# rvolden/C3POa

Hardware: AMD Instinct MI355X
Metric: R2C2 reads->consensus/sec (higher is better)
Workload: dtype int32

## Files before the change

### c3poa_amd/csrc/c3_api.hip

```cpp
#include "c3_dev.h"
#include "c3_args.h"
#include "c3_bgzf.h"
#include "c3_fastq.h"
#include "c3_inflate.h"
#include <algorithm>
#include <cstddef>
#include <cstdio>
#include <cstring>
#include <string>
#include <vector>

extern "C" void c3k_launch_conk(const ConkArgs*, int, int, int, hipStream_t);
extern "C" void c3k_launch_adapter(const AdapterArgs*, int, hipStream_t);
extern "C" void c3k_launch_pairwise(const uint8_t*, int, const uint8_t*, int, const uint8_t*, int, uint8_t*, uint8_t*, int*, hipStream_t);
extern "C" void c3k_launch_match_index(const char*, const int*, int, int, const char*, const long long*, int*, hipStream_t);
extern "C" void c3k_launch_demux(const uint8_t*, int, const uint8_t*, int, int, int, int32_t*, uint8_t*, hipStream_t);
extern "C" void c3k_launch_peaks(const PeaksArgs*, int, hipStream_t);
extern "C" int c3k_peaks_blocks_per_cu(void);
extern "C" void c3k_launch_poa(const PoaArgs*, int, int, int, hipStream_t);
extern "C" void c3k_launch_prep(const PrepArgs*, int, hipStream_t);
extern "C" void c3k_launch_window(const WinArgs*, int, hipStream_t);
extern "C" void c3k_launch_stitch(const StitchArgs*, int, hipStream_t);
extern "C" void c3k_launch_zero(const ZeroArgs*, int, hipStream_t);
extern "C" void c3k_launch_zero_long(const ZeroArgs*, int, hipStream_t);
// ... 494 lines not shown
  }
  HIPCHK(hipMemcpyAsync(h->d_zwork.p, h->zwork.data(), sizeof(int) * (size_t)nz, hipMemcpyHostToDevice, h->stream));
  if (ns) {
    ZeroArgs z; fill_zero_args(h, z, ns); z.dcap = dmax;
    DBG("zero: nz=%d grid=%d dmax=%lld\n", ns, std::min(ns, 512), dmax);
    c3k_launch_zero(&z, std::min(ns, 512), h->stream);
    HIPCHK(hipGetLastError());
  }
  if (nl) {
    ZeroArgs z; fill_zero_args(h, z, nl);
    z.work = h->d_zwork.as<int>() + ns; z.S = h->s_zero_l.as<uint8_t>(); z.scap = smax; z.zk = zk;
    DBG("zero long: nz=%d grid=%d slot=%lld K=%d\n", nl, grid_l, smax, zk);
    c3k_launch_zero_long(&z, grid_l, h->stream);
    HIPCHK(hipGetLastError());
  }
  { int r_ = copy_summary(h); DBG("zero done\n"); return r_; }
}

static int fetch_summary(c3_handle* h) {
  int rc = copy_summary(h);
  DBG("summary copied\n");
  if (rc) return rc;
  const auto wl0 = std::chrono::steady_clock::now();
  struct WlTimer { c3_handle* h; std::chrono::steady_clock::time_point t0; ~WlTimer() { h->tm.ms_host_worklist = std::chrono::duration<float, std::milli>(std::chrono::steady_clock::now() - t0).count(); } } wl_timer_{h, wl0};
  HIPCHK(zero_cnt(h, &dev_cnt(h)->zero_cells));
  if ((rc = run_zero(h))) return rc;
  const int n = h->n;
  h->work.clear();
  for (int i = 0; i < n; ++i) if (h->sum[i].status == C3_ST_OK && h->sum[i].n_sub >= 1) h->work.push_back(i);
  if (n < (1 << 24)) {
    const size_t m = h->work.size();
    std::vector<uint64_t> keys(m), tmp(m);
    for (size_t k = 0; k < m; ++k) {
      const int i = h->work[k];
      const uint64_t cost = (uint64_t)h->sum[i].sum_sub * (uint64_t)h->sum[i].n_sub;
      keys[k] = ((((uint64_t)1 << 40) - 1 - cost) << 24) | (uint64_t)i;
    }
    uint64_t* src = keys.data(); uint64_t* dst = tmp.data();
    for (int pass = 0; pass < 4; ++pass) {
      const int sh = 24 + 10 * pass;
      size_t cnt[1025] = {0};
      for (size_t k = 0; k < m; ++k) ++cnt[((src[k] >> sh) & 1023) + 1];
      for (int b = 0; b < 1024; ++b) cnt[b + 1] += cnt[b];
      for (size_t k = 0; k < m; ++k) dst[cnt[(src[k] >> sh) & 1023]++] = src[k];
      std::swap(src, dst);
    }
    for (size_t k = 0; k < m; ++k) h->work[k] = (int)(src[k] & 0xffffff);
  } else {
    std::stable_sort(h->work.begin(), h->work.end(), [&](int x, int y) {
      long cx = (long)h->sum[x].sum_sub * h->sum[x].n_sub, cy = (long)h->sum[y].sum_sub * h->sum[y].n_sub; return cx > cy; });
  }
  HIPCHK(h->d_work.ensure(sizeof(int) * std::max<size_t>(h->work.size(), 1)));
  if (!h->work.empty()) HIPCHK(hipMemcpyAsync(h->d_work.p, h->work.data(), sizeof(int) * h->work.size(), hipMemcpyHostToDevice, h->stream));
  return 0;
}

static int launch_poa(c3_handle* h, const int* d_work, int nw, int Ncap, int K, int Pcap, long long cells, int* d_overflow, int* d_overflow16, int waves_per_cu, int wide_ring) {
  cells = (cells + 15) & ~15LL;
  cells = (cells + 63) & ~63LL;
  const bool w32 = d_overflow16 == nullptr || getenv("C3_DEBUG_POA32");
  const PoaLayout L = c3_poa_layout(Ncap, K, (int)cells, c3_poa_far_shift(w32), Pcap);
  const int slots = auto_slots(h, h->cfg.slots_poa, L.total, nw, waves_per_cu);
  const size_t S = (size_t)slots;
  HIPCHK(h->s_poa_i.ensure(L.ints * S)); HIPCHK(h->s_poa_nk.ensure(L.edges * S));
  HIPCHK(h->s_poa_cells.ensure(L.cells * S + 256)); HIPCHK(h->s_poa_b.ensure(L.bases * S)); HIPCHK(h->s_poa_sc.ensure(L.score * S));
  HIPCHK(h->s_poa_desc.ensure(L.desc * S)); HIPCHK(h->s_poa_jump.ensure(L.jump * S)); HIPCHK(h->s_poa_path.ensure(L.path * S));
  PoaArgs a; memset(&a, 0, sizeof(a));
  a.b = dev_batch(h); a.info = h->d_info.as<C3Info>(); a.p = dev_params(h->cfg);
  a.cnt = dev_cnt(h); a.work = d_work; a.n_work = nw;
  a.ibase = h->s_poa_i.as<int>(); a.ebase = h->s_poa_nk.as<int>(); a.cellsb = h->s_poa_cells.as<char>();
  a.bbase = h->s_poa_b.as<uint8_t>(); a.score = h->s_poa_sc.as<long long>();
  a.Ncap = Ncap; a.K = K; a.Pcap = Pcap; a.cells_cap = (int)cells; a.desc = h->s_poa_desc.as<uint4>(); a.jump = h->s_poa_jump.as<int>();
  a.pbase = h->s_poa_path.as<int>(); a.overflow = d_overflow; a.overflow16 = d_overflow16;
  if (const char* e = getenv("C3_DEBUG_POA_RBSPAN")) a.rb_span = std::max(3300, atoi(e));
  a.no2col = getenv("C3_DEBUG_POA_NO2COL") != nullptr;
  a.draft = h->d_draft.as<uint8_t>(); a.tpos = h->d_tpos.as<int32_t>();
  a.msa_dbg = nullptr; a.msa_off = nullptr; a.msa_len = nullptr;
  if (h->debug_msa) { a.msa_dbg = h->d_msa.as<uint8_t>(); a.msa_off = h->d_msa_off.as<int64_t>(); a.msa_len = h->d_msa_len.as<int>(); }
  DBG("poa: nw=%d Ncap=%d K=%d cells=%lld slots=%d (%.1f MB per slot)%s\n", nw, Ncap, K, cells, slots, L.total / 1048576.0, d_overflow ? "" : (d_overflow16 ? " [full-size pass]" : " [32-bit pass]"));
  c3k_launch_poa(&a, slots, w32 ? 1 : 0, wide_ring, h->stream);
  HIPCHK(hipGetLastError());
  return 0;
}

static int run_poa(c3_handle* h) {
  const int nw = (int)h->work.size();
  HIPCHK(h->d_draft.ensure((size_t)h->total + 64)); HIPCHK(h->d_tpos.ensure(sizeof(int32_t) * (size_t)h->total + 64));
  HIPCHK(h->d_cons.ensure((size_t)h->total + 64));
  HIPCHK(hipMemsetAsync(h->d_tpos.p, 0xff, sizeof(int32_t) * (size_t)h->total, h->stream));
  if (nw == 0) return 0;
  int max_sum = 0, max_ns = 0, max_q = 0;
  for (int i : h->work) { max_sum = std::max(max_sum, h->sum[i].sum_sub); max_ns = std::max(max_ns, h->sum[i].n_sub); max_q = std::max(max_q, h->sum[i].max_sub); }
  const int Ncap_full = max_sum + 8, K = max_ns + 1, Pcap = max_sum + 8;
  const int w = h->cfg.poa_band_b + (int)(h->cfg.poa_band_f * max_q);
  long long cells_full = (long long)(2 * max_q + 2) * (2 * w + 1 + max_q / 5);
  if (max_ns < 2) cells_full = 64;
  if (cells_full > 0x7fffff00LL) cells_full = 0x7fffff00LL;
  const double nodes_typ = (double)max_q * (1.0 + 0.15 * std::max(0, max_ns - 1));
  int Ncap = (int)std::min<double>(Ncap_full, 1.3 * nodes_typ + 256);
  long long cells = std::min<long long>(cells_full, (long long)(1.5 * nodes_typ * (2 * w + 12)) + 4096);
  if (const char* e_ = getenv("C3_DEBUG_POA_SMALL")) { Ncap = std::min(Ncap_full, std::max(64, atoi(e_))); cells = std::min<long long>(cells_full, 16LL * Ncap); }
  if (h->debug_msa) {
    std::vector<int64_t> mo(h->n + 1, 0);
    for (int i = 0; i < h->n; ++i) mo[i + 1] = mo[i] + (int64_t)h->sum[i].n_sub * (h->sum[i].sum_sub + 2);
    HIPCHK(h->d_msa.ensure((size_t)mo[h->n] + 64)); HIPCHK(h->d_msa_off.ensure(sizeof(int64_t) * (h->n + 1))); HIPCHK(h->d_msa_len.ensure(sizeof(int) * h->n));
    HIPCHK(hipMemcpyAsync(h->d_msa_off.p, mo.data(), sizeof(int64_t) * (h->n + 1), hipMemcpyHostToDevice, h->stream));
    HIPCHK(hipMemsetAsync(h->d_msa_len.p, 0, sizeof(int) * h->n, h->stream));
    HIPCHK(hipStreamSynchronize(h->stream));
  }
  HIPCHK(h->d_overflow.ensure(sizeof(int) * 2 * (size_t)nw));
  C3Counters* dc = dev_cnt(h);
  HIPCHK(zero_cnt(h, &dc->queue)); HIPCHK(zero_cnt(h, &dc->cells)); HIPCHK(zero_cnt(h, &dc->poa_ovf)); HIPCHK(zero_cnt(h, &dc->poa_ovf16));
  HIPCHK(zero_cnt(h, &dc->phases));
  int wide_ring = (max_q > 1792 || 2 * w + 1 + 24 > 128) ? 1 : 0;
  if (const char* e_ = getenv("C3_DEBUG_POA_WIDE")) wide_ring = atoi(e_) ? 1 : 0;
  int* ovA = h->d_overflow.as<int>(); int* ovB = h->d_overflow.as<int>() + nw;
  int rc = launch_poa(h, h->d_work.as<int>(), nw, Ncap, K, Pcap, cells, ovA, ovB, 24, wide_ring);
  if (rc) return rc;
  h->n_poa_redo = 0; h->n_poa_redo16 = 0;
  C3Counters c;
  HIPCHK(read_counters(h, &c));
  if (c.poa_ovf > 0) {
    h->n_poa_redo = c.poa_ovf;
    HIPCHK(zero_cnt(h, &dc->queue));
    if ((rc = launch_poa(h, ovA, c.poa_ovf, Ncap_full, K, Pcap, cells_full, nullptr, ovB, 24, wide_ring))) return rc;
    HIPCHK(read_counters(h, &c));
  }
  if (c.poa_ovf16 > 0) {
    h->n_poa_redo += c.poa_ovf16; h->n_poa_redo16 = c.poa_ovf16;
    HIPCHK(zero_cnt(h, &dc->queue));
    if ((rc = launch_poa(h, ovB, c.poa_ovf16, Ncap_full, K, Pcap, cells_full, nullptr, nullptr, 24, 0))) return rc;
  }
  if (!h->zwork.empty()) {
    ZeroArgs z; fill_zero_args(h, z, (int)h->zwork.size());
    c3k_launch_zero_finish(&z, std::min((int)h->zwork.size(), 512), h->stream);
    HIPCHK(hipGetLastError());
  }
  HIPCHK(hipMemcpyAsync(h->phase_poa, dc->phases, sizeof(h->phase_poa), hipMemcpyDeviceToHost, h->stream));
  return 0;
}

static int run_polish(c3_handle* h, float* ms_prep, float* ms_win, float* ms_st) {
  const int nw = (int)h->work.size();
  DBG("polish: nw=%d\n", nw);
  HIPCHK(h->d_cons.ensure((size_t)h->total + 64));
  if (nw == 0) return 0;
  const int WL = h->cfg.pol_window;
  int max_ns = 0, max_q = 0, max_dang = 0; long long wcap = 0;
  for (int i : h->work) {
    max_ns = std::max(max_ns, h->sum[i].n_sub); max_q = std::max(max_q, h->sum[i].max_sub); max_dang = std::max(max_dang, h->sum[i].max_dang);
    wcap += (2 * h->sum[i].max_sub + WL - 1) / WL + 1;
  }
  const int NLcap = max_ns + 2, NWcap = (2 * max_q + WL - 1) / WL + 1;
  const int64_t ecap = (int64_t)(max_dang + 2) * 512;
  const size_t per_slot_prep = (size_t)ecap + (size_t)NLcap * NWcap * 8;
  const int slots_p = auto_slots(h, h->cfg.slots_poa, per_slot_prep, nw, getenv("C3_DEBUG_PREP_WPC") ? atoi(getenv("C3_DEBUG_PREP_WPC")) : 20);
  HIPCHK(h->s_eD.ensure((size_t)ecap * slots_p));
  HIPCHK(h->s_lw.ensure(sizeof(int) * (size_t)NLcap * NWcap * 2 * slots_p));
  HIPCHK(h->d_wrec.ensure(sizeof(WinRec) * (size_t)wcap)); HIPCHK(h->d_wlay.ensure(sizeof(WLayer) * (size_t)wcap * NLcap));
  HIPCHK(h->d_wbase.ensure(sizeof(int) * (size_t)h->n));
  PrepArgs p; memset(&p, 0, sizeof(p));
  p.b = dev_batch(h); p.info = h->d_info.as<C3Info>(); p.p = dev_params(h->cfg);
  p.cnt = dev_cnt(h); p.work = h->d_work.as<int>(); p.n_work = nw;
  p.draft = h->d_draft.as<uint8_t>(); p.tpos = h->d_tpos.as<int32_t>();
  p.eD = h->s_eD.as<uint8_t>(); p.ecap = ecap;
  p.lw_first = h->s_lw.as<int>(); p.lw_last = p.lw_first + (size_t)NLcap * NWcap * slots_p; p.NLcap = NLcap; p.NWcap = NWcap;
  p.wrec = h->d_wrec.as<WinRec>(); p.wlay = h->d_wlay.as<WLayer>(); p.win_base = h->d_wbase.as<int>();
  p.wcap = (int)std::min<long long>(wcap, 0x7fffffff);
  HIPCHK(zero_counters(h));
  HIPCHK(hipEventRecord(h->ev[5], h->stream));
  DBG("prep: slots=%d ecap=%lld NL=%d NW=%d wcap=%lld\n", slots_p, (long long)ecap, NLcap, NWcap, (long long)wcap);
  c3k_launch_prep(&p, slots_p, h->stream);
  HIPCHK(hipGetLastError());
  HIPCHK(hipEventRecord(h->ev[6], h->stream));
  C3Counters c;
  HIPCHK(read_counters(h, &c));
  h->tm.cells_polish += c.cells; h->tm.cells_polish_computed += c.cells;
  const int n_win = (int)std::min<long long>(c.n_windows, std::min<long long>(wcap, 0x7fffffff));
  h->n_windows = n_win;
  DBG("prep done: n_win=%d\n", n_win);
  const int wout_cap = 3 * WL + 64;
  HIPCHK(hipEventRecord(h->ev[7], h->stream));
  if (n_win > 0) {
    HIPCHK(h->d_wout.ensure((size_t)n_win * wout_cap));
    const int Ncap = 3 * WL + 40 * NLcap, K = NLcap + 2;
    const long long hcap_full = (long long)(Ncap + 1) * 64 * 12;
    const int R_typ = std::min(Ncap, WL + WL / 4 + 30 * NLcap + 64);
    long long hcap = std::min(hcap_full, (long long)(R_typ + R_typ / 2 + 4) * 256);
    if (const char* e = getenv("C3_DEBUG_HCAP_DIV")) hcap = std::max(4096LL, hcap_full / std::max(1, atoi(e)) / 64 * 64);
    const WinLayout L = c3_win_layout(Ncap, K, hcap), L2 = c3_win_layout(Ncap, K, hcap_full);
    const int slots = auto_slots(h, h->cfg.slots_win, L.total, n_win, 20);
    const int slots2 = hcap < hcap_full ? std::min(slots, 256) : 0;
    const size_t S = (size_t)slots, S2 = (size_t)slots2;
    HIPCHK(h->s_win_i.ensure(L.ints * S + 64)); HIPCHK(h->s_win_nk.ensure(L.edges * S));
    HIPCHK(h->s_win_h.ensure(L.H * S)); HIPCHK(h->s_win_d.ensure(L.D * S + 256));
    HIPCHK(h->s_win_b.ensure(L.bases * S)); HIPCHK(h->s_win_sc.ensure(L.score * S)); HIPCHK(h->s_win_desc.ensure(L.desc * S));
    if (slots2) {
      HIPCHK(h->s_win_h2.ensure(L2.H * S2)); HIPCHK(h->s_win_d2.ensure(L2.D * S2 + 256));
      HIPCHK(h->d_wovf.ensure(sizeof(int) * (size_t)n_win));
    }
    WinArgs a; memset(&a, 0, sizeof(a));
    a.b = dev_batch(h); a.p = dev_params(h->cfg); a.cnt = dev_cnt(h); a.n_win = n_win;
    a.wrec_in = h->d_wrec.as<WinRec>(); a.wrec = h->d_wrec.as<WinRec>(); a.wlay = h->d_wlay.as<WLayer>(); a.NLcap = NLcap;
    a.draft = h->d_draft.as<uint8_t>();
    a.ibase = h->s_win_i.as<int>(); a.ebase = h->s_win_nk.as<int>();
    a.base = h->s_win_b.as<uint8_t>(); a.score = h->s_win_sc.as<long long>();
    a.H = h->s_win_h.as<int32_t>(); a.D = h->s_win_d.as<uint16_t>(); a.rdesc = h->s_win_desc.as<uint4>(); a.Ncap = Ncap; a.K = K; a.hcap = hcap; a.Lcap = std::min(std::min(Ncap, 2 * WL + 30 * NLcap), ((getenv("C3_DEBUG_WIN_LDS") ? atoi(getenv("C3_DEBUG_WIN_LDS")) : 6656) - 16) / 6);
    if (const char* e = getenv("C3_DEBUG_WIN_LCAP")) a.Lcap = std::max(64, std::min(Ncap, atoi(e)));
    a.wout = h->d_wout.as<uint8_t>(); a.wout_cap = wout_cap;
    HIPCHK(zero_counters(h));
    if (const char* e = getenv("C3_DEBUG_BAND")) a.band_mode = !strcmp(e, "off") ? 1 : !strcmp(e, "fail") ? 2 : !strcmp(e, "verify") ? 3 : 0;
    a.ovf_list = slots2 ? h->d_wovf.as<int>() : nullptr;
    c3k_launch_window(&a, slots, h->stream);
    HIPCHK(hipGetLastError());
    if (slots2) {
      a.H = h->s_win_h2.as<int32_t>(); a.D = h->s_win_d2.as<uint16_t>(); a.hcap = hcap_full;
      a.wlist = h->d_wovf.as<int>(); a.ovf_list = nullptr;
      c3k_launch_window(&a, slots2, h->stream);
      HIPCHK(hipGetLastError());
    }
    HIPCHK(hipMemcpyAsync(h->phase_win, dev_cnt(h)->phases, sizeof(h->phase_win), hipMemcpyDeviceToHost, h->stream));
  }
  HIPCHK(hipEventRecord(h->ev[8], h->stream));
  StitchArgs s; memset(&s, 0, sizeof(s));
  s.b = dev_batch(h); s.info = h->d_info.as<C3Info>(); s.work = h->d_work.as<int>(); s.n_work = nw;
  s.wrec = h->d_wrec.as<WinRec>(); s.win_base = h->d_wbase.as<int>(); s.wout = h->d_wout.as<uint8_t>(); s.wout_cap = wout_cap;
  s.cons = h->d_cons.as<char>(); s.zflag = h->d_zflag.as<uint8_t>();
  DBG("stitch\n");
  c3k_launch_stitch(&s, std::min(nw, h->n_cus * 16), h->stream);
  HIPCHK(hipGetLastError());
  HIPCHK(hipEventRecord(h->ev[9], h->stream));
  HIPCHK(read_counters(h, &c));
  if (n_win > 0) {
    h->tm.n_win_redo = c.win_ovf; h->tm.cells_polish += c.cells; h->tm.cells_polish_computed += c.cells_computed;
    h->tm.n_band_layers = c.band_layers; h->tm.n_band_fallback = c.band_fallback; h->tm.n_band_mismatch = c.band_mismatch;
    if (c.band_mismatch) fprintf(stderr, "c3poa: band verify mismatch in window %d layer %d (R = %d): last differing base q = %d, band row %d, full row %d, row of q+1 = %d\n",
                                 c.verify.window, c.verify.layer, c.verify.R, c.verify.q, c.verify.band_row, c.verify.full_row, c.verify.next_row);
  }
  HIPCHK(hipEventElapsedTime(ms_prep, h->ev[5], h->ev[6]));
  HIPCHK(hipEventElapsedTime(ms_win, h->ev[7], h->ev[8]));
  HIPCHK(hipEventElapsedTime(ms_st, h->ev[8], h->ev[9]));
  h->tm.n_windows = n_win;
  return 0;
}

static const long long QV_BUDGET = 1LL << 30;
static int qv_scratch(c3_handle* h, long long max_m, long long max_n, int n_items, QvArgs& a, int* grid) {
  a.dir_words = (max_m + 7) / 8 * 64;
  a.lds_n = (int)std::min<long long>((max_n + 15) / 16 * 16, c3k_qv_lds_max());
  a.gcap = max_n > a.lds_n ? (max_n + 15) / 16 * 16 : 0;
  const long long per_wg = 4 * 4 * a.dir_words + 5 * a.gcap;
  *grid = (int)std::max(1LL, std::min<long long>(std::min(n_items, h->n_cus * 8), QV_BUDGET / per_wg));
  HIPCHK(h->s_qv_dirs.ensure(sizeof(uint32_t) * (size_t)a.dir_words * 4 * (size_t)*grid + 256));
  if (a.gcap) HIPCHK(h->s_qv_g.ensure((size_t)a.gcap * 5 * (size_t)*grid + 256));
  a.dirs = h->s_qv_dirs.as<uint32_t>();
  a.gS = a.gcap ? h->s_qv_g.as<int>() : nullptr; a.gcodes = a.gcap ? h->s_qv_g.as<uint8_t>() + (size_t)a.gcap * 4 * (size_t)*grid : nullptr;
  HIPCHK(h->d_qv_cnt.ensure(64));
  HIPCHK(hipMemsetAsync(h->d_qv_cnt.p, 0, 64, h->stream));
  a.cnt = h->d_qv_cnt.as<unsigned long long>();
  return 0;
}
static int qv_counts(c3_handle* h, float ms) {
  unsigned long long c[8];
  HIPCHK(hipMemcpyAsync(c, h->d_qv_cnt.p, 64, hipMemcpyDeviceToHost, h->stream));
  HIPCHK(hipStreamSynchronize(h->stream));
  h->qtm.ms_qv = ms; h->qtm.n_reads = (int64_t)c[0]; h->qtm.n_pieces = (int64_t)c[1]; h->qtm.n_skipped = (int64_t)c[2];
  h->qtm.band_cells = (int64_t)c[3]; h->qtm.edge_hits = (int64_t)c[4];
  return 0;
}

static int run_qv(c3_handle* h) {
  for (int i = 0; i < 2; ++i) if (!h->ev_qv[i]) HIPCHK(hipEventCreate(&h->ev_qv[i]));
  HIPCHK(h->d_qv.ensure((size_t)h->total + 64));
  QvArgs a; memset(&a, 0, sizeof(a));
  int grid = 0;
  int rc = qv_scratch(h, h->maxL, h->maxL, h->n, a, &grid);
  if (rc) return rc;
  a.n_reads = h->n; a.info = h->d_info.as<C3Info>(); a.pk = h->d_pk.as<uint32_t>(); a.woff = h->d_woff.as<int64_t>();
  a.qual = h->d_qual.as<uint8_t>(); a.off = h->d_off.as<int64_t>(); a.cons = h->d_cons.as<char>(); a.qv = h->d_qv.as<char>();
  a.sa_np = -1;
  DBG("qv: grid=%d dir_words=%lld lds_n=%d gcap=%lld\n", grid, a.dir_words, a.lds_n, a.gcap);
  HIPCHK(hipEventRecord(h->ev_qv[0], h->stream));
  c3k_launch_qv(&a, grid, h->stream);
  HIPCHK(hipGetLastError());
  HIPCHK(hipEventRecord(h->ev_qv[1], h->stream));
  HIPCHK(hipEventSynchronize(h->ev_qv[1]));
  float ms = 0; HIPCHK(hipEventElapsedTime(&ms, h->ev_qv[0], h->ev_qv[1]));
  return qv_counts(h, ms);
}

extern "C" int c3_batch_run(c3_handle* h, int stages) {
  if (!h || h->n <= 0) return C3_E_STATE;
  if ((stages & C3_STAGE_QV) && !((stages | h->stages_done) & C3_STAGE_POLISH))
    return c3_fail(h, C3_E_STATE, "C3_STAGE_QV needs the polish stage (in this call or an earlier one on the resident batch)");
  HIPCHK(hipSetDevice(h->cfg.device));
  int rc;
  float ms;
  hipEvent_t t0 = h->ev[0], t1 = h->ev[1], t2 = h->ev[2], t3 = h->ev[3], t4 = h->ev[4];
  DBG("run: start n=%d\n", h->n);
  const auto wall0 = std::chrono::steady_clock::now();
  const double alloc0 = g_alloc_ms;
  if (stages & C3_STAGE_CONK) { h->tm.ms_conk = 0; h->tm.cells_conk = 0; }
  if (stages & C3_STAGE_PEAKS) h->tm.ms_peaks = 0;
  if (stages & C3_STAGE_POA) { h->tm.ms_poa = 0; h->tm.cells_poa = 0; }
  if (stages & C3_STAGE_POLISH) { h->tm.ms_prep = h->tm.ms_window = h->tm.ms_stitch = 0; h->tm.cells_polish = 0; h->tm.cells_polish_computed = 0; h->tm.n_band_layers = h->tm.n_band_fallback = h->tm.n_band_mismatch = 0; h->tm.n_windows = 0; h->tm.n_win_redo = 0; }
  HIPCHK(hipEventRecord(t0, h->stream));
  if (stages & C3_STAGE_CONK) { if ((rc = run_conk(h))) return rc; h->tm.cells_conk = 0; for (int i = 0; i < h->n; ++i) h->tm.cells_conk += (h->off[i + 1] - h->off[i]) * (int64_t)h->max_spl; }
// ... 915 lines not shown
```

### c3poa_amd/csrc/k_polish.hip

```cpp
#include "c3_dev.h"
#include "c3_args.h"
#include <algorithm>

#define WSYNC() __syncthreads()
#define EI(v, k) ((size_t)(k) * (size_t)c.Ncap + (size_t)(v))
#ifndef C3_WIN_RING
#define C3_WIN_RING 1
#endif



#ifndef C3_PREP_WAVES
#define C3_PREP_WAVES 5
#endif
#define EC 5
#define EXT_DCAP 4096
template <bool DL>
__device__ long long extend_align(const PrepArgs& a, const uint32_t* pk, const uint8_t* draft, const uint8_t* ldraft, int C,
                                  int pb, int n, int dir_, int32_t* tpos, uint8_t* D, int lane) {
  const int W = a.p.dang_band, bw = 2 * W + 1;
  const int mt4 = a.p.pol_match * 4, mm4 = a.p.pol_mismatch * 4, g4 = a.p.pol_gap * 4;
  const int db = dir_ > 0 ? 0 : C - 1;
  const int NEGK = -(1 << 28);
  for (int k = lane; k < n; k += 64) tpos[pb + dir_ * k] = -1;
  if (bw > 64 * EC || (long long)(n + 1) * 512 > a.ecap) return -1;
  int hprev[EC];
#pragma unroll
  for (int cc = 0; cc < EC; ++cc) {
    const int bb = lane * EC + cc, j = bb - W;
    hprev[cc] = (bb < bw && j >= 0 && j <= C) ? j * g4 : NEGK;
  }
  int best = 0, bi = 0, bj = 0;
  long long cells = lane == 0 ? min(C, W) + 1 : 0;
#ifndef C3_EXT_OLD
  if (DL) {
    const int bb0 = lane * EC;
    int g4bb1[EC], bestc[EC], bic[EC];
#pragma unroll
    for (int cc = 0; cc < EC; ++cc) { g4bb1[cc] = g4 * (bb0 + cc) + 1; bestc[cc] = 0; bic[cc] = 0; }
    auto code_at = [&](int q) { return (unsigned)ldraft[db + dir_ * min(max(q, 0), C - 1)]; };
    unsigned dcp = 0;
#pragma unroll
    for (int cc = 0; cc < EC; ++cc) dcp |= code_at(1 - W + bb0 + cc - 1) << (4 * cc);
    long long cells_s = 0;
    for (int ib = 1; ib <= n; ib += 64) {
      int pcs = 0;
      if (ib + lane <= n) pcs = c3_code_at(pk, pb + dir_ * (ib + lane - 1));
      asm volatile("" : "+v"(pcs));
      const int cnt = min(64, n - ib + 1);
      for (int li = 0; li < cnt; ++li) {
        const int i = ib + li;
        const int pc = __builtin_amdgcn_readlane(pcs, li);
        const unsigned nxt_code = code_at(i - W + bb0 + EC - 1);
        const int vlo = W - i;
        const int vhi = min(bw - 1, C - i + W);
        const unsigned span = (unsigned)(vhi - vlo);
        cells_s += max(0, vhi - max(0, vlo) + 1);
        const int nxt0 = __builtin_amdgcn_update_dpp(NEGK, hprev[0], 0x130, 0xf, 0xf, false);
        int key[EC], y[EC];
        int run = NEGK;
#pragma unroll
        for (int cc = 0; cc < EC; ++cc) {
          const int dcode = (int)((dcp >> (4 * cc)) & 15u);
          const int kd = hprev[cc] + ((pc == dcode) ? mt4 + 3 : mm4 + 3);
          const int up = (cc + 1 < EC) ? hprev[cc + 1 < EC ? cc + 1 : cc] : nxt0;
          const int k = max(kd, up + (g4 + 2));
          const bool val = (unsigned)(bb0 + cc - vlo) <= span && vhi >= vlo && bb0 + cc >= 0;
          key[cc] = val ? k : NEGK;
          y[cc] = (key[cc] & ~3) - (g4bb1[cc] - 1);
          run = max(run, y[cc]);
        }
        const int s = wave_scan_max(run);
        int ex = wave_shr1(s, NEGK);
        unsigned d0 = 0, d1 = 0;
#pragma unroll
        for (int cc = 0; cc < EC; ++cc) {
          int k2 = max(key[cc], ex + g4bb1[cc]);
          ex = max(ex, y[cc]);
          k2 = key[cc] == NEGK ? NEGK : k2;
          const int hh = k2 & ~3;
          hprev[cc] = hh;
          const unsigned tag = (unsigned)k2 & 3u;
          if (cc < 4) d0 |= tag << (8 * cc); else d1 |= tag;
          const bool up_ = hh > bestc[cc];
          bestc[cc] = max(bestc[cc], hh);
          bic[cc] = up_ ? i : bic[cc];
        }
        unsigned* drow = (unsigned*)(D + (size_t)i * 512) + lane * 2;
        drow[0] = 0x03030303u - d0; drow[1] = 3u - d1;
        dcp = (dcp >> 4) | (nxt_code << (4 * (EC - 1)));
      }
    }
#pragma unroll
    for (int cc = 0; cc < EC; ++cc) {
      const bool better = bestc[cc] > best || (bestc[cc] == best && bestc[cc] > 0 && bic[cc] < bi);
      if (better) { best = bestc[cc]; bi = bic[cc]; bj = bic[cc] - W + bb0 + cc; }
    }
    cells += lane == 0 ? cells_s : 0;
  } else
#endif
  for (int ib = 1; ib <= n; ib += 64) {
    int pcs = 0;
    if (ib + lane <= n) pcs = c3_code_at(pk, pb + dir_ * (ib + lane - 1));
    asm volatile("" : "+v"(pcs));
    const int cnt = min(64, n - ib + 1);
    for (int li = 0; li < cnt; ++li) {
      const int i = ib + li;
      const int pc = __builtin_amdgcn_readlane(pcs, li);
      const int jlo = max(0, i - W);
      const int nxt0 = __builtin_amdgcn_update_dpp(NEGK, hprev[0], 0x130, 0xf, 0xf, false);
      int key[EC], y[EC];
      int run = NEGK;
#pragma unroll
      for (int cc = 0; cc < EC; ++cc) {
        const int bb = lane * EC + cc, j = i - W + bb;
        const bool val = bb < bw && j >= 0 && j <= C;
        int k = INT32_MIN;
        if (val) {
          if (j > 0) {
            const int dcode = DL ? (int)ldraft[db + dir_ * (j - 1)] : (int)draft[db + dir_ * (j - 1)];
            k = hprev[cc] + ((pc == dcode) ? mt4 : mm4) + 3;
          }
          const int up = (cc + 1 < EC) ? hprev[cc + 1 < EC ? cc + 1 : cc] : nxt0;
          if (bb + 1 < bw) k = max(k, up + g4 + 2);
        }
        key[cc] = val ? k : NEGK;
        y[cc] = val ? (k & ~3) - g4 * bb : NEGK;
        run = max(run, y[cc]);
      }
      const int s = wave_scan_max(run);
      int ex = wave_shr1(s, NEGK);
      unsigned d0 = 0, d1 = 0;
#pragma unroll
      for (int cc = 0; cc < EC; ++cc) {
        const int bb = lane * EC + cc, j = i - W + bb;
        const bool val = bb < bw && j >= 0 && j <= C;
        int k2 = key[cc];
        if (val && j > jlo) k2 = max(k2, ex + g4 * bb + 1);
        ex = max(ex, y[cc]);
        const int hh = k2 & ~3;
        hprev[cc] = val ? hh : NEGK;
        const unsigned dir = val ? (unsigned)(3 - (k2 & 3)) : 3u;
        if (cc < 4) d0 |= dir << (8 * cc); else d1 |= dir;
        if (val) { ++cells; if (j > 0 && hh > best) { best = hh; bi = i; bj = j; } }
      }
      unsigned* drow = (unsigned*)(D + (size_t)i * 512) + lane * 2;
      drow[0] = d0; drow[1] = d1;
    }
  }
  WSYNC();
  const int gb = wave_max(best);
  const int gi = wave_min(best == gb ? bi : INT32_MAX / 2);
  const int gj = wave_min((best == gb && bi == gi) ? bj : INT32_MAX / 2);
  if (gb > 0) {
    int i = gi, j = gj;
    while (i > 0 || j > 0) {
      if (i == 0) break;
      const int bb = j - i + W;
      const int ik = i - lane;
      int d = 3;
      if (ik >= 1) d = D[(size_t)ik * 512 + (bb / EC) * 8 + bb % EC];
      const unsigned long long bal = __ballot(ik >= 1 && d == 0 && j - lane >= 1);
      const int m = (~bal) ? __builtin_ctzll(~bal) : 64;
      if (lane < m) tpos[pb + dir_ * (ik - 1)] = db + dir_ * (j - lane - 1);
      i -= m; j -= m;
      if (m < 64 && i > 0) {
        const int dbk = wave_bcast(d, m);
        if (dbk == 1) --i; else if (dbk == 2) --j; else break;
      }
    }
  }
  WSYNC();
  long long tot = cells;
  for (int o = 32; o > 0; o >>= 1) tot += __shfl_xor(tot, o);
  return tot;
}

__device__ __forceinline__ void prep_one(const PrepArgs& a, int wi, int lane, uint8_t* ldraft, uint8_t* eD, int* lwf, int* lwl, int WL) {
    const int rid = a.work[wi];
    C3Info* info = &a.info[rid];
    if (info->status != C3_ST_OK || info->draft_len <= 0) { info->n_win = 0; a.win_base[rid] = 0; return; }
    const int64_t off = a.b.off[rid];
    const int L = (int)(a.b.off[rid + 1] - off);
    const uint32_t* pk = a.b.pk + a.b.woff[rid];
    const uint8_t* qual = a.b.qual + off;
    const uint8_t* draft = a.draft + off;
    int32_t* tpos = a.tpos + off;
    const int C = info->draft_len, ns = info->n_sub;
    const int hf = info->has_front, ht = info->has_tail;
    long long cells = 0;
    if ((ht || hf) && C <= EXT_DCAP) { for (int t = lane; t < C; t += 64) ldraft[t] = draft[t]; WSYNC(); }
#ifdef C3_EXP_X2_EXT
    if (C <= EXT_DCAP) {
      if (ht) { long long r = extend_align<true>(a, pk, draft, ldraft, C, info->tail_beg, L - info->tail_beg, +1, tpos, eD, lane); if (r > 1LL << 60) cells += r; }
      if (hf) { long long r = extend_align<true>(a, pk, draft, ldraft, C, info->front_end - 1, info->front_end, -1, tpos, eD, lane); if (r > 1LL << 60) cells += r; }
    }
#endif
    if (C <= EXT_DCAP) {
      if (ht) { long long r = extend_align<true>(a, pk, draft, ldraft, C, info->tail_beg, L - info->tail_beg, +1, tpos, eD, lane); if (r > 0) cells += r; }
      if (hf) { long long r = extend_align<true>(a, pk, draft, ldraft, C, info->front_end - 1, info->front_end, -1, tpos, eD, lane); if (r > 0) cells += r; }
    } else {
      if (ht) { long long r = extend_align<false>(a, pk, draft, ldraft, C, info->tail_beg, L - info->tail_beg, +1, tpos, eD, lane); if (r > 0) cells += r; }
      if (hf) { long long r = extend_align<false>(a, pk, draft, ldraft, C, info->front_end - 1, info->front_end, -1, tpos, eD, lane); if (r > 0) cells += r; }
    }
    const int nl = ns + hf + ht;
    const int nwin = (C + WL - 1) / WL;
    if (nwin > a.NWcap || nl > a.NLcap) { info->status = C3_ST_LIMIT; info->n_win = 0; a.win_base[rid] = 0; return; }
    long tl = 0;
    for (int i = 0; i < nl; ++i) {
      int lb, le;
      if (i < ns) { lb = info->sub_beg[i]; le = info->sub_end[i]; }
      else if (i == ns && hf) { lb = 0; le = info->front_end; }
      else { lb = info->tail_beg; le = L; }
      tl += le - lb;
    }
    const int tgs = tl > 1000L * nl;
    int wbase = 0;
    if (lane == 0) wbase = atomicAdd(&a.cnt->n_windows, nwin);
    wbase = wave_first(wbase);
    if (wbase + nwin > a.wcap) {
      for (int w = lane; w < nwin && wbase + w < a.wcap; w += 64) {
        WinRec r; r.rid = rid; r.w = w; r.n_layers = 0; r.blen = 0; r.tgs = 0; r.out_len = 0; r.polished = 0; r.pad_ = 0;
        a.wrec[wbase + w] = r;
      }
      info->status = C3_ST_LIMIT; info->n_win = 0; a.win_base[rid] = 0; return;
    }
    for (int i = lane; i < nl * nwin; i += 64) { lwf[i] = INT32_MAX; lwl[i] = -1; }
    for (int w = lane; w < nwin; w += 64) {
      WinRec r; r.rid = rid; r.w = w; r.n_layers = 0; r.blen = (w * WL + WL <= C) ? WL : C - w * WL; r.tgs = tgs; r.out_len = 0; r.polished = 0; r.pad_ = 0;
      a.wrec[wbase + w] = r;
    }
    WSYNC();
    for (int i = 0; i < nl; ++i) {
      int lb, le;
      if (i < ns) { lb = info->sub_beg[i]; le = info->sub_end[i]; }
      else if (i == ns && hf) { lb = 0; le = info->front_end; }
      else { lb = info->tail_beg; le = L; }
      int qf = INT32_MAX, ql = -1;
      for (int k0 = lb; k0 < le; k0 += 64) {
        const int k = k0 + lane;
        const int t = k < le ? tpos[k] : -1;
        const bool valid = t >= 0;
        const int w = valid ? t / WL : -1;
        const unsigned long long vm = __ballot(valid);
        const unsigned long long below = vm & ((1ull << lane) - 1ull);
        const unsigned long long above = lane == 63 ? 0ull : (vm & ~((2ull << lane) - 1ull));
        const int pl = below ? 63 - __builtin_clzll(below) : lane, nx = above ? __builtin_ctzll(above) : lane;
        const int wp = __shfl(w, pl), wn = __shfl(w, nx);
        if (valid) {
          qf = min(qf, k); ql = max(ql, k);
          if (!below || wp != w) atomicMin(&lwf[i * nwin + w], k);
          if (!above || wn != w) atomicMax(&lwl[i * nwin + w], k);
        }
      }
      qf = wave_min(qf); ql = wave_max(ql);
      WSYNC();
      if (ql < 0) continue;
      const int qs = ql + 1 - qf, ts = tpos[ql] + 1 - tpos[qf];
      const double err = 1.0 - (double)min(qs, ts) / (double)max(qs, ts);
      if (err > 0.3) continue;
      for (int w = 0; w < nwin; ++w) {
        const int fq = lwf[i * nwin + w], lq = lwl[i * nwin + w];
        if (lq < 0) continue;
        const int seglen = lq + 1 - fq;
        if ((double)seglen < 0.02 * WL) continue;
        long qsum = 0;
        for (int x = fq + lane; x <= lq; x += 64) qsum += (int)qual[x] - 33;
        for (int o = 32; o > 0; o >>= 1) qsum += __shfl_xor(qsum, o);
        if (qsum < (long)a.p.pol_q * seglen) continue;
        if (lane == 0) {
          WinRec* r = &a.wrec[wbase + w];
          WLayer* dst = &a.wlay[(size_t)(wbase + w) * a.NLcap + r->n_layers];
          dst->qbeg = fq; dst->len = seglen; dst->begin = tpos[fq] - w * WL; dst->end = tpos[lq] - w * WL;
          r->n_layers++;
        }
      }
      WSYNC();
    }
    if (lane == 0) {
      info->n_win = nwin; a.win_base[rid] = wbase;
      atomicAdd(&a.cnt->cells, (unsigned long long)cells);
    }
    WSYNC();
}

__global__ __launch_bounds__(64, C3_PREP_WAVES) void k_prep(PrepArgs a) {
  const int lane = wave_lane();
  const int slot = blockIdx.x;
  __shared__ uint8_t ldraft[EXT_DCAP];
  uint8_t* eD = a.eD + (size_t)slot * a.ecap;
  int* lwf = a.lw_first + (size_t)slot * a.NLcap * a.NWcap;
  int* lwl = a.lw_last + (size_t)slot * a.NLcap * a.NWcap;
  const int WL = a.p.pol_window;
  for (;;) {
    int wi = 0;
    if (lane == 0) wi = atomicAdd(&a.cnt->queue, 1);
    wi = wave_first(wi);
    if (wi >= a.n_work) break;
    prep_one(a, wi, lane, ldraft, eD, lwf, lwl, WL);
  }
}


template <class T> struct WArr {
  T* base; unsigned off;
  __device__ __forceinline__ T& at(unsigned i) const { return *(T*)((char*)base + ((i + off) * (unsigned)sizeof(T))); }
  __device__ __forceinline__ T& operator[](int i) const { return at((unsigned)i); }
  __device__ __forceinline__ T& operator[](unsigned i) const { return at(i); }
  __device__ __forceinline__ T& operator[](long long i) const { return at((unsigned)i); }
  __device__ __forceinline__ T& operator[](size_t i) const { return at((unsigned)i); }
  __device__ __forceinline__ T* ptr() const { return base + off; }
};
#define W_QCAP 704
#define W_TBW 448
// ... 1044 lines not shown
```

Measured before the change: 416,900.

## Pack extend-align traceback directions into 2-bit fields and read query words via scalar loads

After: 419,000, median of 6. About the same (+0.5%).

```diff
diff --git a/c3poa_amd/csrc/c3_api.hip b/c3poa_amd/csrc/c3_api.hip
--- a/c3poa_amd/csrc/c3_api.hip
+++ b/c3poa_amd/csrc/c3_api.hip
@@ -670,7 +670,7 @@
     wcap += (2 * h->sum[i].max_sub + WL - 1) / WL + 1;
   }
   const int NLcap = max_ns + 2, NWcap = (2 * max_q + WL - 1) / WL + 1;
-  const int64_t ecap = (int64_t)(max_dang + 2) * 512;
+  const int64_t ecap = (int64_t)(max_dang + 2) * 128;
   const size_t per_slot_prep = (size_t)ecap + (size_t)NLcap * NWcap * 8;
   const int slots_p = auto_slots(h, h->cfg.slots_poa, per_slot_prep, nw, getenv("C3_DEBUG_PREP_WPC") ? atoi(getenv("C3_DEBUG_PREP_WPC")) : 20);
   HIPCHK(h->s_eD.ensure((size_t)ecap * slots_p));
diff --git a/c3poa_amd/csrc/k_polish.hip b/c3poa_amd/csrc/k_polish.hip
--- a/c3poa_amd/csrc/k_polish.hip
+++ b/c3poa_amd/csrc/k_polish.hip
@@ -23,7 +23,7 @@
   const int db = dir_ > 0 ? 0 : C - 1;
   const int NEGK = -(1 << 28);
   for (int k = lane; k < n; k += 64) tpos[pb + dir_ * k] = -1;
-  if (bw > 64 * EC || (long long)(n + 1) * 512 > a.ecap) return -1;
+  if (bw > 64 * EC || (long long)(n + 1) * 128 > a.ecap) return -1;
   int hprev[EC];
 #pragma unroll
   for (int cc = 0; cc < EC; ++cc) {
@@ -43,14 +43,17 @@
 #pragma unroll
     for (int cc = 0; cc < EC; ++cc) dcp |= code_at(1 - W + bb0 + cc - 1) << (4 * cc);
     long long cells_s = 0;
-    for (int ib = 1; ib <= n; ib += 64) {
-      int pcs = 0;
-      if (ib + lane <= n) pcs = c3_code_at(pk, pb + dir_ * (ib + lane - 1));
-      asm volatile("" : "+v"(pcs));
-      const int cnt = min(64, n - ib + 1);
-      for (int li = 0; li < cnt; ++li) {
-        const int i = ib + li;
-        const int pc = __builtin_amdgcn_readlane(pcs, li);
+    int lo2 = lane * 2;
+    asm volatile("" : "+v"(lo2));
+    uint8_t* drow = D + 128 + lo2;
+    typedef const __attribute__((address_space(4))) uint32_t* cpk_t;
+    const cpk_t pkc = (cpk_t)pk;
+    auto word_of = [&](int i) { return pkc[__builtin_amdgcn_readfirstlane((pb + dir_ * (i - 1)) >> 4)]; };
+    unsigned pws = word_of(1);
+    {
+      for (int i = 1; i <= n; ++i) {
+        const int pc = (int)((pws >> (((pb + dir_ * (i - 1)) & 15) * 2)) & 3u);
+        pws = word_of(min(i + 1, n));
         const unsigned nxt_code = code_at(i - W + bb0 + EC - 1);
         const int vlo = W - i;
         const int vhi = min(bw - 1, C - i + W);
@@ -72,7 +75,7 @@
         }
         const int s = wave_scan_max(run);
         int ex = wave_shr1(s, NEGK);
-        unsigned d0 = 0, d1 = 0;
+        unsigned dw = 0;
 #pragma unroll
         for (int cc = 0; cc < EC; ++cc) {
           int k2 = max(key[cc], ex + g4bb1[cc]);
@@ -81,13 +84,13 @@
           const int hh = k2 & ~3;
           hprev[cc] = hh;
           const unsigned tag = (unsigned)k2 & 3u;
-          if (cc < 4) d0 |= tag << (8 * cc); else d1 |= tag;
+          dw |= tag << (2 * cc);
           const bool up_ = hh > bestc[cc];
           bestc[cc] = max(bestc[cc], hh);
           bic[cc] = up_ ? i : bic[cc];
         }
-        unsigned* drow = (unsigned*)(D + (size_t)i * 512) + lane * 2;
-        drow[0] = 0x03030303u - d0; drow[1] = 3u - d1;
+        *(uint16_t*)drow = (uint16_t)(0x3ffu - dw);
+        drow += 128;
         dcp = (dcp >> 4) | (nxt_code << (4 * (EC - 1)));
       }
     }
@@ -130,7 +133,7 @@
       }
       const int s = wave_scan_max(run);
       int ex = wave_shr1(s, NEGK);
-      unsigned d0 = 0, d1 = 0;
+      unsigned dw = 0;
 #pragma unroll
       for (int cc = 0; cc < EC; ++cc) {
         const int bb = lane * EC + cc, j = i - W + bb;
@@ -141,11 +144,10 @@
         const int hh = k2 & ~3;
         hprev[cc] = val ? hh : NEGK;
         const unsigned dir = val ? (unsigned)(3 - (k2 & 3)) : 3u;
-        if (cc < 4) d0 |= dir << (8 * cc); else d1 |= dir;
+        dw |= dir << (2 * cc);
         if (val) { ++cells; if (j > 0 && hh > best) { best = hh; bi = i; bj = j; } }
       }
-      unsigned* drow = (unsigned*)(D + (size_t)i * 512) + lane * 2;
-      drow[0] = d0; drow[1] = d1;
+      ((uint16_t*)(D + (size_t)i * 128))[lane] = (uint16_t)dw;
     }
   }
   WSYNC();
@@ -159,7 +161,7 @@
       const int bb = j - i + W;
       const int ik = i - lane;
       int d = 3;
-      if (ik >= 1) d = D[(size_t)ik * 512 + (bb / EC) * 8 + bb % EC];
+      if (ik >= 1) d = (((const uint16_t*)(D + (size_t)ik * 128))[bb / EC] >> (2 * (bb % EC))) & 3;
       const unsigned long long bal = __ballot(ik >= 1 && d == 0 && j - lane >= 1);
       const int m = (~bal) ? __builtin_ctzll(~bal) : 64;
       if (lane < m) tpos[pb + dir_ * (ik - 1)] = db + dir_ * (j - lane - 1);
```
